# saitejasrivilli/movie-recommender-demo

Measured on AMD Instinct MI355X. Metric: end-to-end recs/sec (1M ads d=256, top-500->10), higher is better.
Workload: dtype f32 (f16x3 emulation: 2 fp16 planes per operand, 3 fp16-MFMA products per MAC, fp32 accumulate)

## Files before the change

### include/amdrec.h

```cpp
#ifndef AMDREC_H
#define AMDREC_H
#include <stddef.h>
#include <stdint.h>

#ifdef __cplusplus
extern "C" {
#endif

#define AMDREC_ABI_VERSION 14
#define AMDREC_MAX_K 2048

int amdrec_abi_version(void);
const char* amdrec_last_error(void);

int amdrec_flat_search_workspace(int64_t nq, int64_t nrows, int k, size_t* bytes );
int amdrec_flat_search(const float* corpus, int64_t nrows, int64_t ld_corpus, int dim,
                       const float* queries, int64_t nq, int64_t ld_queries, int k,
                       int64_t pos_offset, float* out_scores ,
                       int64_t* out_pos , void* workspace, size_t workspace_bytes,
                       int* n_fixup, void* stream);

int amdrec_bf16_rows(const float* x, int64_t rows, int64_t ld, int dim, uint16_t* out ,
                     int64_t ld_out, float* max_norm , void* stream);
int amdrec_flat_search_mixed_workspace(int64_t nq, int64_t nrows, int k, int dim, size_t* bytes );
// ... 201 lines not shown
    const int32_t* table_off;
    const int32_t* cards;
    const float* w_proj;
    const float* b_proj;
    const float* w_proj_user;
    const float* w_proj_ad;
    int32_t ldw_proj_user, ldw_proj_ad;
    amdrec_encoder_layer layers[AMDREC_MAX_LAYERS];
    const float* cross_wt[AMDREC_MAX_LAYERS];
    const float* cross_b[AMDREC_MAX_LAYERS];
    const float* head_w1;
    const float* head_b1;
    const float* head_w2[AMDREC_MAX_TASKS];
    const float* head_b2[AMDREC_MAX_TASKS];
    const float* head_w3[AMDREC_MAX_TASKS];
    const float* head_b3[AMDREC_MAX_TASKS];
    const float* ad_proj_cache;
    int64_t ld_ad_proj_cache;
    const float* ad_hidden_cache;
    int64_t ld_ad_hidden_cache;
    const uint16_t* cross_wt_x6[AMDREC_MAX_LAYERS];
    const uint16_t* head_w1_x6;
    amdrec_x3_weights x3;
} amdrec_ranker_params;

int amdrec_ranker_workspace(const amdrec_ranker_params* p , int64_t rows, size_t* bytes );
int amdrec_ranker_forward(const amdrec_ranker_params* p , const int64_t* user_cat,
                          const float* numerical, int64_t user_rowdiv, const int64_t* ad_cat,
                          const int64_t* ad_rowmap, int64_t rows, float* out_logits, int64_t ld_logits,
                          int* bad_index_flag, int64_t n_user_rows, int64_t n_ad_rows, void* workspace,
                          size_t workspace_bytes, void* stream);

int amdrec_ranker_forward_ctr_first(const amdrec_ranker_params* p , const int64_t* user_cat,
                                    const float* numerical, int64_t user_rowdiv, const int64_t* ad_cat,
                                    const int64_t* ad_rowmap, int64_t rows, float* out_logits ,
                                    int64_t ld_logits, int* bad_index_flag, int64_t n_user_rows, int64_t n_ad_rows,
                                    float* trunk_out , int64_t ld_trunk, void* workspace,
                                    size_t workspace_bytes, void* stream);
int amdrec_ranker_ctr_first_supported(const amdrec_ranker_params* p , int64_t rows);
int amdrec_ranker_winner_heads(const amdrec_ranker_params* p , const float* trunk ,
                               int64_t ld_trunk, int64_t n_trunk_rows, const int32_t* slots ,
                               int64_t n_users, int k_c, int top_k, float* out_scores ,
                               void* workspace, size_t workspace_bytes, void* stream);
int amdrec_ranker_ctr_first_workspace(const amdrec_ranker_params* p , int64_t rows, int64_t n_winner_rows,
                                      size_t* bytes );

// ... 76 lines not shown
```

### movie-recommender-demo_amd/amdrec/ranker.py

```python
from __future__ import annotations

from typing import Dict, List, NamedTuple, Optional, Tuple

import torch
import torch.nn as nn

from . import _lib, weights


class _Attention(nn.Module):
    def __init__(self, d_model, num_heads, dropout):
        super().__init__()
        assert d_model % num_heads == 0
        self.d_model, self.num_heads, self.d_k = d_model, num_heads, d_model // num_heads
        for n in ("W_q", "W_k", "W_v", "W_o"):
            setattr(self, n, nn.Linear(d_model, d_model))
        self.dropout = nn.Dropout(dropout)


class _FFN(nn.Module):
    def __init__(self, d_model, d_ff, dropout):
        super().__init__()
        self.fc1, self.fc2 = nn.Linear(d_model, d_ff), nn.Linear(d_ff, d_model)
        self.dropout = nn.Dropout(dropout)
# ... 49 lines not shown
        super().__init__()
        self.user_embeddings = nn.ModuleDict({n: nn.Embedding(c, embedding_dim) for n, c in user_feature_dims.items()})
        self.ad_embeddings = nn.ModuleDict({n: nn.Embedding(c, embedding_dim) for n, c in ad_feature_dims.items()})
        total = (len(user_feature_dims) + len(ad_feature_dims)) * embedding_dim + numerical_dim
        self.feature_projection = nn.Linear(total, d_model)
        self.positional_encoding = nn.Parameter(torch.randn(1, max_seq_len, d_model))
        self.transformer_layers = nn.ModuleList([_EncoderLayer(d_model, num_heads, d_ff, dropout)
                                                 for _ in range(num_layers)])
        self.feature_interaction = _Cross(d_model, 3, dropout)
        self.prediction_heads = nn.ModuleDict({t: _head(d_model, dropout) for t in ("ctr", "engagement", "revenue")})
        self.d_model = d_model
        self.dropout = nn.Dropout(dropout)
        self._user_names, self._ad_names, self._n_num = list(user_feature_dims), list(ad_feature_dims), numerical_dim
        self._packed = None
        self._ad_cache = None
        self.fuse_attention = True
        self.fold_first_attention = True
        self.cache_first_ffn = True
        self.hidden_cache_max_bytes = 8 << 30
        self.gemm_engine = "f16x3"
        self.x3_min_rows = 1
        self.x3_variant = 16
        self.x3_cs_max_rows = 0

    ENGINES = ("f16x3", "bf16x6", "fp32")
    SMALL_ROWS = 8192

    def x3_fallback_reason(self):
        return weights.x3_ineligible_reason(self.state_dict(), self.fuse_attention)

    def ctr_first_unsupported_reason(self):
        key = (self.gemm_engine, self.fuse_attention, int(self.x3_variant), int(self.x3_min_rows), _lib._REG_EPOCH[0])
        c = self.__dict__.get("_ctr_first_why")
        if c is None or c[0] != key:
            c = self.__dict__["_ctr_first_why"] = (key, self._ctr_first_unsupported_reason())
        return c[1]

    def _ctr_first_unsupported_reason(self):
        if self.gemm_engine != "f16x3":
            return f"gemm_engine {self.gemm_engine!r} (the mode runs on the f16x3 row-owner kernels only)"
        why = self.x3_fallback_reason()
        if why is not None:
            return f"not the row-owner engine's architecture ({why})"
        if int(self.x3_variant) != 16:
            return f"x3_variant {self.x3_variant} (the 32-row kernel has no task window and no gathered input)"
        if int(self.x3_min_rows) != 1:
# ... 99 lines not shown
                out = hid[n_old:]
                _lib.check(lib.amdrec_ranker_project_ads_hidden(
                    _lib.C.byref(params), _lib.ptr(tail), n_new - n_old, _lib.ptr(out), hid.stride(0), _lib.ptr(ws),
                    ws.numel(), _lib.stream_ptr(dev)))
        self._ad_cache = _AdCache(c.key, *_table_key(new_table), proj, hid)

    def _entry_for(self, table) -> Optional[_AdCache]:
        c = getattr(self, "_ad_cache", None)
        if c is None or self._packed is None or c.key != self._packed.key or c[1:4] != _table_key(table):
            return None
        return c

    def _cache_for(self, table):
        return getattr(self._entry_for(table), "proj", None)

    def _hidden_cache_for(self, table):
        return getattr(self._entry_for(table), "hidden", None)

    def _pack(self, device):
        if self.gemm_engine not in self.ENGINES:
            raise ValueError(f"gemm_engine must be one of {self.ENGINES}")
        key = (str(device), self.fuse_attention, bool(self.fold_first_attention), bool(self.cache_first_ffn),
               self.gemm_engine, int(self.x3_min_rows), int(self.x3_variant), int(self.x3_cs_max_rows),
               _lib.tensor_versions(self))
        if self._packed is None or self._packed.key != key:
            sd = self.state_dict()
            why = weights.x3_ineligible_reason(sd, self.fuse_attention) if self.gemm_engine == "f16x3" else None
            x3 = self.gemm_engine == "f16x3" and why is None
            if why is not None:
                import warnings
                warnings.warn(f"amdrec TransformerRanker: gemm_engine 'f16x3' is not available for these weights ({why}); "
                              f"running the generic tile GEMMs (bf16x6 above {self.SMALL_ROWS} rows, fp32 MFMA below)",
                              RuntimeWarning, stacklevel=3)
            self._packed = _Packed(key, *weights.pack_ranker(
                sd, self._user_names, self._ad_names, self._n_num, device, fuse_attention=self.fuse_attention,
                x6=self.gemm_engine == "bf16x6" or (self.gemm_engine == "f16x3" and not x3), x3=x3,
                x3_min_rows=self.x3_min_rows, x3_variant=self.x3_variant, x3_cs_max_rows=self.x3_cs_max_rows,
                fold_first_attention=bool(self.fold_first_attention), cache_first_ffn=bool(self.cache_first_ffn)))
        return self._packed.params, self._packed.tasks

    def load_state_dict(self, state_dict, *a, **k):
        r = super().load_state_dict(state_dict, *a, **k)
        self.invalidate()
        return r

    def autograd_forward(self, user_categorical, ad_categorical, numerical, mask=None):
        import math
        F = torch.nn.functional
        ue = torch.cat([e(user_categorical[:, i].long()) for i, e in enumerate(self.user_embeddings.values())], dim=1)
        ae = torch.cat([e(ad_categorical[:, i].long()) for i, e in enumerate(self.ad_embeddings.values())], dim=1)
        x = self.feature_projection(torch.cat([ue, ae, numerical], dim=1)).unsqueeze(1)
        x = self.dropout(x + self.positional_encoding[:, :1, :])
        for layer in self.transformer_layers:
            at = layer.self_attention
            B = x.size(0)
            q = at.W_q(x).view(B, -1, at.num_heads, at.d_k).transpose(1, 2)
            k = at.W_k(x).view(B, -1, at.num_heads, at.d_k).transpose(1, 2)
            v = at.W_v(x).view(B, -1, at.num_heads, at.d_k).transpose(1, 2)
            scores = torch.matmul(q, k.transpose(-2, -1)) / math.sqrt(at.d_k)
            if mask is not None:
                scores = scores.masked_fill(mask == 0, -1e9)
# ... 150 lines not shown
```

### movie-recommender-demo_amd/amdrec/weights.py

```python
from __future__ import annotations

import ctypes as C
from typing import Dict, List, NamedTuple

import numpy as np
import torch

MAX_LAYERS = 8
MAX_TASKS = 4
_FP = C.c_void_p
TASKS = ("ctr", "engagement", "revenue")


class TowerParams(C.Structure):
    _fields_ = [("n_feat", C.c_int32), ("emb_dim", C.c_int32), ("n_num", C.c_int32), ("n_layers", C.c_int32),
                ("dims", C.c_int32 * (MAX_LAYERS + 1)), ("ldw", C.c_int32 * MAX_LAYERS),
                ("tables", _FP), ("table_off", _FP), ("cards", _FP),
                ("w", _FP * MAX_LAYERS), ("b", _FP * MAX_LAYERS), ("renormalize", C.c_int32)]


class EncoderLayer(C.Structure):
    _fields_ = [(n, _FP) for n in ("w_v", "b_v", "w_o", "b_o", "ln1_g", "ln1_b", "w_1", "b_1", "w_2", "b_2",
                                   "ln2_g", "ln2_b")] + [("ldw_dm", C.c_int32), ("ldw_ff", C.c_int32)] + \
               [(n, _FP) for n in ("w_o_x6", "w_1_x6", "w_2_x6")]
# ... 8 lines not shown
                ("stream_cs", _FP), ("chunks_cs", C.c_int64), ("cs_max_rows", C.c_int64), ("fold_attn1", C.c_int64),
                ("stream_hc", _FP), ("chunks_hc", C.c_int64), ("params_hc", _FP), ("w_user_uq", _FP), ("b_user_uq", _FP),
                ("w_hidden_ad", _FP),
                ("stream_ctr", _FP), ("chunks_ctr", C.c_int64), ("stream_ctr_cs", _FP), ("chunks_ctr_cs", C.c_int64),
                ("stream_ctr_hc", _FP), ("chunks_ctr_hc", C.c_int64), ("stream_win", _FP), ("chunks_win", C.c_int64),
                ("stream_win_cs", _FP), ("chunks_win_cs", C.c_int64)]


class RankerParams(C.Structure):
    _fields_ = [("n_user_feat", C.c_int32), ("n_ad_feat", C.c_int32), ("emb_dim", C.c_int32), ("n_num", C.c_int32),
                ("d_model", C.c_int32), ("d_ff", C.c_int32), ("n_layers", C.c_int32), ("n_cross", C.c_int32),
                ("n_tasks", C.c_int32), ("head_h1", C.c_int32), ("head_h2", C.c_int32), ("ln_eps", C.c_float),
                ("ldw_proj", C.c_int32), ("ldw_cross", C.c_int32), ("ldw_head1", C.c_int32),
                ("ldw_head2", C.c_int32),
                ("tables", _FP), ("table_off", _FP), ("cards", _FP), ("w_proj", _FP), ("b_proj", _FP),
                ("w_proj_user", _FP), ("w_proj_ad", _FP), ("ldw_proj_user", C.c_int32), ("ldw_proj_ad", C.c_int32),
                ("layers", EncoderLayer * MAX_LAYERS),
                ("cross_wt", _FP * MAX_LAYERS), ("cross_b", _FP * MAX_LAYERS),
                ("head_w1", _FP), ("head_b1", _FP),
                ("head_w2", _FP * MAX_TASKS), ("head_b2", _FP * MAX_TASKS),
                ("head_w3", _FP * MAX_TASKS), ("head_b3", _FP * MAX_TASKS),
                ("ad_proj_cache", _FP), ("ld_ad_proj_cache", C.c_int64),
                ("ad_hidden_cache", _FP), ("ld_ad_hidden_cache", C.c_int64),
                ("cross_wt_x6", _FP * MAX_LAYERS), ("head_w1_x6", _FP), ("x3", X3Weights)]


def _np64(t):
    if isinstance(t, torch.Tensor):
        return t.detach().cpu().double().numpy()
    return np.asarray(t, dtype=np.float64)


def split_planes(w32: np.ndarray) -> np.ndarray:
    w = np.ascontiguousarray(w32, dtype=np.float32)
    out_f, ld = w.shape
    assert ld % 32 == 0
    u = w.view(np.uint32)
    h = (u & np.uint32(0xffff0000)).view(np.float32)
    r1 = w - h
    m = (r1.view(np.uint32) & np.uint32(0xffff0000)).view(np.float32)
    r2 = r1 - m
    planes = np.stack([(x.view(np.uint32) >> np.uint32(16)).astype(np.uint16) for x in (h, m, r2)], axis=0)
    assert np.array_equal(h + m + r2, w)
    return np.ascontiguousarray(planes.reshape(3, out_f, ld // 16, 16).transpose(1, 2, 0, 3)).view(np.int16)


X3_TARGET_EXP = 12
# ... 91 lines not shown
    for t in range(T + 1):
        for u in range(8):
            if t < T:
                out += _pair(f1, 2 * t, u)
            if t >= 1:
                out += _pair(f2, 2 * u, t - 1)
    return np.stack(out)


def x3b_stream_ffn_stage2(f2):
    out = []
    for t in range(f2.shape[1]):
        for u in range(8):
            out += _pair(f2, 2 * u, t)
    return np.stack(out)


def _task_window(f2s, tiles_per_task, tasks):
    t0, n = (0, len(f2s)) if tasks is None else tasks
    assert 0 <= t0 and n >= 1 and t0 + n <= len(f2s)
    return f2s[t0:t0 + n], t0 * tiles_per_task


def x3b_stream_heads(f1, f2s, tiles_per_task, tasks=None):
    f2s, base = _task_window(f2s, tiles_per_task, tasks)
    nt = len(f2s) * tiles_per_task
    assert nt % 2 == 0 and (nt * 10) % 4 == 0, "head stream is not a whole number of chunks"
    out = []
    for tt in range(nt + 1):
        prev = tt - 1
        for u in range(8):
            if tt < nt:
                out += _pair(f1, 2 * (base + tt), u)
            if tt >= 1 and u in (3, 7):
                out += _pair(f2s[prev // tiles_per_task], 2 * (u // 4), prev % tiles_per_task)
    return np.stack(out)


def _wave_chunk(groups):
    out = []
    for g in groups:
        out += g if g is not None else [np.zeros((64, 8), np.uint16)] * 4
    assert len(out) == 16
    return out


def x3c_stream_gemm256(fr):
    assert fr.shape[0] == 16
    out = []
    for ks in range(fr.shape[1]):
        for j in range(2):
# ... 83 lines not shown

def x3_hidden_bound(w1: np.ndarray, b1: np.ndarray):
    return float(16.0 * np.linalg.norm(w1, axis=1).max() * (1 + 1e-6)), float(np.abs(b1).max())


def x3_split(mats: Dict, variant: int = 32, fold_first: bool = False):
    mats, lift = x3_rebalance(mats)
    frags = x3_frags if variant == 32 else x3b_frags
    fr, sc = {"tiles": mats["h1"].shape[0] // len(mats["h2"]) // 32}, {}
    for name, dst in (("ov", "sw_ov"), ("w1", "sw_1"), ("w2", "sw_2"), ("cross", "sw_cross")):
        ws = [None if name == "ov" and fold_first and l == 0 else w for l, w in enumerate(mats[name])]
        sc[dst] = [1.0 if w is None else x3_pow2_scale(np.abs(w).max()) for w in ws]
        fr[name] = [None if w is None else frags(w, s) for w, s in zip(ws, sc[dst])]
    sc["sw_h1"] = x3_pow2_scale(np.abs(mats["h1"]).max())
    sc["sw_h2"] = x3_pow2_scale(max(np.abs(w).max() for w in mats["h2"]))
    fr["h1"], fr["h2"] = frags(mats["h1"], sc["sw_h1"]), [frags(w, sc["sw_h2"]) for w in mats["h2"]]
    bounds = [x3_hidden_bound(w, b) for w, b in zip(mats["w1"], mats["b1"])]
    sc["hn"], sc["hb"] = [n for n, _ in bounds], [b for _, b in bounds]
    sc["hn_head"], sc["hb_head"] = x3_hidden_bound(mats["h1"], mats["hb1"])
    sc["lift"] = lift
    return fr, sc


def x3_order(fr: Dict, kind, cache_first_ffn: bool = False, tasks=None, trunk: bool = True) -> np.ndarray:
    s_gemm, s_cross, s_ffn, s_heads = _X3_ORDER[kind]
    assert trunk or not cache_first_ffn
    assert tasks is None or kind in (16, "16cs"), "task windows exist for the 16-row kernels only"
    parts = []
    for l, (ov, f1, f2) in enumerate(zip(fr["ov"], fr["w1"], fr["w2"]) if trunk else ()):
        parts += [] if ov is None else [s_gemm(ov)]
        parts.append(x3b_stream_ffn_stage2(f2) if cache_first_ffn and l == 0 else s_ffn(f1, f2))
    parts += [s_cross(f) for f in fr["cross"]] if trunk else []
    parts.append(s_heads(fr["h1"], fr["h2"], fr["tiles"], *(() if tasks is None else (tasks,))))
    stream = np.concatenate(parts)
    assert stream.shape[0] % 16 == 0 and (kind != "16cs" or all(len(q) % 64 == 0 for q in parts))
    return stream


def x3_ctr_first_orders(n_tasks: int, column_split: bool, cache_first_ffn: bool) -> Dict:
    win = (1, n_tasks - 1)
    orders = {"ctr": dict(kind=16, tasks=(0, 1)), "win": dict(kind=16, tasks=win, trunk=False)}
    if column_split:
        orders["ctr_cs"] = dict(kind="16cs", tasks=(0, 1))
        orders["win_cs"] = dict(kind="16cs", tasks=win, trunk=False)
    if cache_first_ffn:
        orders["ctr_hc"] = dict(kind=16, tasks=(0, 1), cache_first_ffn=True)
    return orders


def pack_x3_stream(mats: Dict, variant: int = 32, fold_first: bool = False, cache_first_ffn: bool = False) -> Dict:
    assert variant in (16, 32, "16cs")
    assert not cache_first_ffn or (variant == 16 and fold_first)
    fr, sc = x3_split(mats, variant, fold_first)
    stream = x3_order(fr, variant, cache_first_ffn)
    return {"stream": stream, "chunks": stream.shape[0] // 16, **sc}

# ... 184 lines not shown
        L.w_o, L.ldw_dm, L.w_o_x6 = pk.mat(c["wov"], x6)
    else:
        L.b_v = pk.vec(c["bv"])
        L.w_v, L.ldw_dm, _ = pk.mat(c["wv"])
        L.w_o, L.ldw_dm, L.w_o_x6 = pk.mat(c["wo"], x6)
    L.w_1, L.ldw_dm, L.w_1_x6 = pk.mat(c["w1"], x6)
    L.b_o = pk.vec(c["b_ov"] if fuse_attention else c["bo"])
    L.w_2, L.ldw_ff, L.w_2_x6 = pk.mat(c["w2"], x6)
    for dst, src in (("b_1", "b1"), ("b_2", "b2"), ("ln1_g", "g1"), ("ln1_b", "be1"), ("ln2_g", "g2"), ("ln2_b", "be2")):
        setattr(L, dst, pk.vec(c[src]))


def _pack_x3(p: RankerParams, pk: Packed, ch: RankerChain, wproj, bproj, nu: int, na: int, cache_first_ffn: bool):
    f32 = lambda a: a.astype(np.float32).astype(np.float64)
    fold = bool(p.x3.fold_attn1)
    mats = {"ov": [f32(L["wov"]) for L in ch.layers], "w1": [f32(L["w1"]) for L in ch.layers],
            "b1": [f32(L["b1"]) for L in ch.layers], "w2": [f32(L["w2"]) for L in ch.layers],
            "cross": [f32(w) for w in ch.cross_wt], "h1": f32(ch.head_w1), "hb1": f32(ch.head_b1),
            "h2": [f32(h["w2"]) for h in ch.heads]}
    fr, sc = x3_split(mats, p.x3.variant, fold)
    pk.x3_fragments = fr

    def stream(kind, **kw):
        s = x3_order(fr, kind, **kw)
        return pk.ptr(s.view(np.int16)), s.shape[0] // 16
    lift = sc["lift"]
    layers = [dict(L, b1=_scaled(L["b1"], f)) for L, f in zip(ch.layers, lift["w1"])]
    heads = [dict(h, b2=_scaled(h["b2"], f), w3=_scaled(h["w3"], 1.0 / f)) for h, f in zip(ch.heads, lift["h2"])]
    blob = pack_x3_params(layers, ch.cross_b, _scaled(ch.head_b1, lift["h1"]), heads, fold_first=fold)
    assert len(blob) <= X3_PARAM_FLOATS
    p.x3.params, p.x3.n_params = pk.ptr(blob), len(blob)
    p.x3.stream, p.x3.chunks = stream(p.x3.variant)
    if p.x3.cs_max_rows >= 0 and x3c_available(p):
        p.x3.stream_cs, p.x3.chunks_cs = stream("16cs")
    if cache_first_ffn and x3_hidden_cache(p):
        hc = first_ffn_cache(ch, nu, na, folded=(wproj, bproj), lift=lift["w1"][0])
        p.x3.stream_hc, p.x3.chunks_hc = stream(16, cache_first_ffn=True)
        blob_hc = blob.copy()
        blob_hc[512:512 + len(hc["c"])] = hc["c"].astype(np.float32)
        p.x3.params_hc = pk.ptr(blob_hc)
        p.x3.w_user_uq, ldu, _ = pk.mat(np.concatenate([_user_ad_columns(wproj, nu, na)[0], hc["w_user"]]))
        p.x3.b_user_uq = pk.vec(np.concatenate([bproj, hc["b"]]))
        p.x3.w_hidden_ad, lda, _ = pk.mat(hc["w_ad"])
        assert ldu == p.ldw_proj_user and lda == p.ldw_proj_ad
    for dst in ("sw_ov", "sw_1", "sw_2", "hn", "hb", "sw_cross"):
        for i, v in enumerate(sc[dst]):
            getattr(p.x3, dst)[i] = v
    p.x3.sw_h1, p.x3.sw_h2, p.x3.hn_head, p.x3.hb_head = sc["sw_h1"], sc["sw_h2"], sc["hn_head"], sc["hb_head"]


def ctr_first_packable(p: RankerParams) -> bool:
    return bool(p.x3.stream) and p.x3.variant == 16 and p.n_tasks >= 2


def pack_ctr_first(p: RankerParams, pk: Packed) -> bool:
    if p.x3.stream_ctr:
        return True
    fr = getattr(pk, "x3_fragments", None)
    if fr is None or not ctr_first_packable(p):
        return False
    for stem, kw in x3_ctr_first_orders(p.n_tasks, bool(p.x3.stream_cs), bool(p.x3.stream_hc)).items():
        s = x3_order(fr, **kw)
        setattr(p.x3, "stream_" + stem, pk.ptr(s.view(np.int16)))
        setattr(p.x3, "chunks_" + stem, s.shape[0] // 16)
    return True


def pack_ranker(sd: Dict, user_names: List[str], ad_names: List[str], n_num: int, device, ln_eps=1e-5,
                fuse_attention: bool = True, x6: bool = True, x3: bool = False, x3_min_rows: int = 0,
                x3_variant: int = 32, x3_cs_max_rows: int = 0, fold_first_attention: bool = False,
                cache_first_ffn: bool = False):
    pk = Packed(device)
    tables = [sd[f"user_embeddings.{n}.weight"] for n in user_names] + \
             [sd[f"ad_embeddings.{n}.weight"] for n in ad_names]
    p = RankerParams()
    p.tables, p.table_off, p.cards, emb_dim = pack_tables(pk, tables)
    ch = ranker_chain(sd)
    if len(ch.layers) > MAX_LAYERS:
        raise ValueError(f"at most {MAX_LAYERS} encoder layers are supported (num_layers > {MAX_LAYERS})")
    x3 = bool(x3) and x3_eligible(sd, fuse_attention)
    fold = bool(fold_first_attention and x3 and int(x3_min_rows) == 1 and ch.layers)
    wproj, bproj = folded_projection(ch) if fold else (ch.w_proj, ch.b_proj)
    assert wproj.shape[1] == len(tables) * emb_dim + n_num
    p.n_user_feat, p.n_ad_feat, p.emb_dim, p.n_num = len(user_names), len(ad_names), emb_dim, n_num
    p.d_model, p.ln_eps = wproj.shape[0], ln_eps
    p.w_proj, p.ldw_proj, _ = pk.mat(wproj)
    nu, na = len(user_names) * emb_dim, len(ad_names) * emb_dim
    if nu + n_num > 0 and na > 0:
        w_user, w_ad = _user_ad_columns(wproj, nu, na)
        p.w_proj_user, p.ldw_proj_user, _ = pk.mat(w_user)
        p.w_proj_ad, p.ldw_proj_ad, _ = pk.mat(w_ad)
    p.b_proj = pk.vec(bproj)
    for l, c in enumerate(ch.layers):
        _pack_encoder_layer(p.layers[l], pk, c, fuse_attention, x6)
    p.n_layers, p.n_cross, p.n_tasks = len(ch.layers), len(ch.cross_wt), len(ch.tasks)
    p.d_ff = ch.layers[-1]["w1"].shape[0] if ch.layers else 4
    for c, (w, b) in enumerate(zip(ch.cross_wt, ch.cross_b)):
        p.cross_wt[c], p.ldw_cross, p.cross_wt_x6[c] = pk.mat(w, x6)
        p.cross_b[c] = pk.vec(b)
    p.head_h1, p.head_h2 = ch.head_w1.shape[0] // len(ch.tasks), ch.heads[0]["w2"].shape[0]
    p.head_w1, p.ldw_head1, p.head_w1_x6 = pk.mat(ch.head_w1, x6)
    p.head_b1 = pk.vec(ch.head_b1)
    for i, h in enumerate(ch.heads):
        p.head_w2[i], p.ldw_head2, _ = pk.mat(h["w2"])
        p.head_b2[i], p.head_w3[i], p.head_b3[i] = pk.vec(h["b2"]), pk.vec(h["w3"]), pk.vec(h["b3"])
    if x3:
        p.x3.variant, p.x3.fold_attn1 = x3_variant, int(fold)
        p.x3.min_rows, p.x3.cs_max_rows = int(x3_min_rows), int(x3_cs_max_rows)
        _pack_x3(p, pk, ch, wproj, bproj, nu, na, cache_first_ffn)
    return p, pk, ch.tasks
```

### movie-recommender-demo_amd/csrc/ranker_x3.hip

```cpp
#include "rowowner.hpp"
#include "rowowner16.hpp"
#include "rowowner16c.hpp"
#include "../../include/amdrec.h"

using namespace amdrec;

static bool x3_folded(const amdrec_ranker_params* p) { return p->x3.fold_attn1 != 0; }
static long long x3_param_floats(const amdrec_ranker_params* p) {
    const long long n = (long long)p->n_layers * (6 * 256 + p->d_ff) + 256ll * p->n_cross + (long long)p->n_tasks * (p->head_h1 + 132) -
                        (x3_folded(p) ? 256 : 0);
    return (n + 1023) / 1024 * 1024;
}

static bool x3_eligible(const amdrec_ranker_params* p) {
    if (p->x3.stream == nullptr || p->x3.chunks <= 0 || p->x3.params == nullptr) return false;
    if (p->x3.variant != 16 && p->x3.variant != 32) return false;
    if (x3_param_floats(p) > x3::PARAM_FLOATS) return false;
    if (p->d_model != 256 || (p->n_layers > 0 && p->d_ff % 32 != 0) || p->head_h1 % 32 != 0 || p->head_h2 != 64) return false;
    if (2 * p->n_layers + p->n_cross + 1 > x3::MAX_PHASES || p->n_tasks > 4) return false;
    for (int l = 0; l < p->n_layers; ++l)
        if (p->layers[l].w_v != nullptr) return false;
    if (x3_folded(p) && (p->n_layers < 1 || p->x3.min_rows != 1)) return false;
    return true;
}

static bool x3c_available(const amdrec_ranker_params* p) {
    return p->x3.variant == 16 && p->x3.stream_cs != nullptr && p->x3.chunks_cs > 0 &&
           (p->n_layers == 0 || p->d_ff % 128 == 0) && p->head_h1 % 128 == 0;
}

constexpr long long X3B4_MAX_ROWS = 256ll * 64;

enum class X3Shape { Rows32x128, Rows16x128, Rows16x64, ColSplit };
static X3Shape x3_shape(const amdrec_ranker_params* p, long long rows) {
    const long long cs_rows = p->x3.cs_max_rows > 0 ? p->x3.cs_max_rows : (p->x3.cs_max_rows < 0 ? 0 : x3c::MAX_ROWS);
    if (x3c_available(p) && rows <= cs_rows) return X3Shape::ColSplit;
    if (p->x3.variant != 16) return X3Shape::Rows32x128;
    return rows <= X3B4_MAX_ROWS ? X3Shape::Rows16x64 : X3Shape::Rows16x128;
}

static bool x3_hidden_cache(const amdrec_ranker_params* p, X3Shape shape) {
    return x3_folded(p) && shape == X3Shape::Rows16x128 && p->x3.stream_hc != nullptr && p->x3.chunks_hc > 0 &&
// ... 30 lines not shown
        if (l == 0 && fold) {
            A.type = x3::PH_LN; A.gamma = o; A.beta = o + 256; A.sw1 = 1.f; A.sw2 = 1.f; A.ln_eps = p->ln_eps;
            o += 512;
        } else {
            A.type = x3::PH_ATTN_LN; A.b1 = o; A.gamma = o + 256; A.beta = o + 512; A.sw1 = p->x3.sw_ov[l];
            A.sw2 = 1.f; A.ln_eps = p->ln_eps;
            o += 768;
        }
        x3::Phase& F = G.ph[n++];
        F.type = hc && l == 0 ? x3::PH_FFN_LN_CACHED : x3::PH_FFN_LN; F.n_steps = p->d_ff / 32; F.b1 = o; F.b2 = o + p->d_ff; F.gamma = o + p->d_ff + 256;
        F.beta = o + p->d_ff + 512;
        F.sw1 = p->x3.sw_1[l]; F.sw2 = p->x3.sw_2[l]; F.hn = p->x3.hn[l]; F.hb = p->x3.hb[l]; F.ln_eps = p->ln_eps;
        o += p->d_ff + 768;
    }
    for (int c = 0; c < p->n_cross; ++c) {
        if (win.heads_only) { o += 256; continue; }
        x3::Phase& C = G.ph[n++];
        C.type = x3::PH_CROSS; C.b1 = o; C.sw1 = p->x3.sw_cross[c]; C.sw2 = 1.f;
        o += 256;
    }
    x3::Phase& H = G.ph[n++];
    H.type = x3::PH_HEADS; H.n_steps = p->head_h1 / 32; H.n_tasks = win.n_tasks; H.b1 = o + win.first_task * p->head_h1;
    H.sw1 = p->x3.sw_h1; H.sw2 = p->x3.sw_h2; H.hn = p->x3.hn_head; H.hb = p->x3.hb_head;
    o += p->n_tasks * p->head_h1;
    for (int t = 0; t < p->n_tasks; ++t) {
        const int i = t - win.first_task;
        if (i >= 0 && i < win.n_tasks) { G.hb2[i] = o; G.hw3[i] = o + 64; G.hb3[i] = o + 128; }
        o += 132;
    }
    REQUIRE(p->x3.n_params == x3_param_floats(p), "x3: parameter blob has %lld floats, the architecture needs %lld",
            (long long)p->x3.n_params, x3_param_floats(p));
    G.params = hc ? p->x3.params_hc : p->x3.params;
    G.n_params = (int)p->x3.n_params;
    const long long per_layer = 16 + 4ll * (p->d_ff / 32);
    const long long hidden_tiles = (long long)win.n_tasks * (p->head_h1 / 32);
    const long long heads = cs ? hidden_tiles * 3 : hidden_tiles * 40 / 16;
    REQUIRE(cs || hidden_tiles * 40 % 16 == 0, "x3: head stream is not a whole number of chunks");
    REQUIRE(!cs || hidden_tiles % 4 == 0, "x3: column-split head stream is not a whole number of super-steps");
    const long long trunk = p->n_layers * per_layer - (fold ? 16 : 0) - (hc ? 2ll * (p->d_ff / 32) : 0) + 16ll * p->n_cross;
    const long long total = (win.heads_only ? 0 : trunk) + heads;
    const amdrec_x3_weights& w = p->x3;
    const void* stream = all_tasks ? (cs ? w.stream_cs : (hc ? w.stream_hc : w.stream))
                         : ctr_first ? (cs ? w.stream_ctr_cs : (hc ? w.stream_ctr_hc : w.stream_ctr))
                                     : (cs ? w.stream_win_cs : w.stream_win);
    const long long have = all_tasks ? (cs ? w.chunks_cs : (hc ? w.chunks_hc : w.chunks))
                           : ctr_first ? (cs ? w.chunks_ctr_cs : (hc ? w.chunks_ctr_hc : w.chunks_ctr))
                                       : (cs ? w.chunks_win_cs : w.chunks_win);
    REQUIRE(stream != nullptr, "x3: the stream of this program is not packed");
    REQUIRE(total == have, "x3: stream length %lld chunks does not match the architecture (%lld)", have, total);
    G.n_phases = n_phases < 0 || n_phases > n ? n : n_phases;
    G.total_chunks = (int)total;
    G.stream = reinterpret_cast<const unsigned char*>(stream);
    return AMDREC_OK;
}

static double x3_weight_elements(const x3::Program& G) {
    double w = 0;
    for (int i = 0; i < G.n_phases; ++i) {
        const x3::Phase& P = G.ph[i];
        if (P.type == x3::PH_ATTN_LN || P.type == x3::PH_CROSS) w += 256.0 * 256.0;
// ... 206 lines not shown
```

### movie-recommender-demo_amd/csrc/rowowner16_impl.hpp

```cpp

#pragma clang diagnostic push
#pragma clang diagnostic ignored "-Wuninitialized-const-reference"
namespace amdrec {
namespace AMDREC_X3B_NAMESPACE {

using x3::CHUNK_BYTES, x3::CHUNK_FRAGS, x3::DBG, x3::f16x8, x3::FRAG_BYTES, x3::Input, x3::lds_byte, x3::lds_cfloat, x3::Phase,
    x3::Program, x3::RING_BYTES;
using x16::add_rows, x16::group6, x16::hidden_planes, x16::init_pair, x16::layer_norm, x16::layer_norm_scaled, x16::load_rows,
    x16::param4, x16::prepare, x16::reduce_sum4, x16::row_scale, x16::split8, x16::store_rows;

#if !defined(AMDREC_X3B_WAVES) || !defined(AMDREC_X3B_NAMESPACE)
#error "include rowowner16.hpp, not this file"
#endif
constexpr int WAVES = AMDREC_X3B_WAVES, ROWS_PER_WAVE = 16, ROWS_PER_WG = WAVES * ROWS_PER_WAVE;
constexpr int DMA_PER_WAVE = CHUNK_FRAGS / WAVES;
constexpr bool PAIRED = WAVES == 8 && !(DBG & (256 | 512));
constexpr int NBUF = PAIRED ? x3::NBUF - 1 : x3::NBUF, DEPTH = NBUF - 3;
constexpr int PAIR_BYTES = CHUNK_BYTES / 4;
constexpr int DMA_GROUP = 1;

struct Ring {
    lds_byte* lds_dma;
    lds_byte* lds_rd;
    int issued, total;
// ... 488 lines not shown

template <bool S1, bool S2, int P0, int GI>
__device__ __forceinline__ void heads_groups(Ring& ring, f16x8 (&cur)[4], const f16x8 (&xh)[8], const f16x8 (&xl)[8],
                                             f32x4& a10, f32x4& a11, f32x4 (&acc2)[4], const f16x8& hh, const f16x8& hl) {
    constexpr int NG = (S1 ? 8 : 0) + (S2 ? 2 : 0);
    constexpr bool is2 = S2 && (!S1 || GI == 4 || GI == 9);
    constexpr int u = !S1 ? 0 : (S2 ? (GI < 4 ? GI : GI - 1) : GI);
    constexpr int pr = !S1 ? GI : (GI == 9 ? 1 : 0);
    f16x8 nxt[4];
    if constexpr (GI < NG - 1) ring.read4<(P0 + GI + 1) & 3>(nxt);
    ring.timed_landed(cur);
    if constexpr (is2) group6(cur, hh, hl, acc2[2 * pr], acc2[2 * pr + 1]);
    else group6(cur, xh[u], xl[u], a10, a11);
    if constexpr (GI < NG - 1) heads_groups<S1, S2, P0, GI + 1>(ring, nxt, xh, xl, a10, a11, acc2, hh, hl);
}
template <bool S1, bool S2, int P0>
__device__ __forceinline__ void heads_step(Ring& ring, const f16x8 (&xh)[8], const f16x8 (&xl)[8], f32x4& a10, f32x4& a11,
                                           f32x4 (&acc2)[4], const f16x8& hh, const f16x8& hl) {
    f16x8 cur[4];
    ring.read4<P0>(cur);
    heads_groups<S1, S2, P0, 0>(ring, cur, xh, xl, a10, a11, acc2, hh, hl);
}

__device__ __forceinline__ void phase_heads(Ring& ring, const Program& G, const Phase& P, const f32x4 (&x)[16], float* out,
                                            long long ld_out, long long row, bool row_ok, int g, lds_cfloat* pb) {
    float s, inv;
    row_scale(x, s, inv);
    f16x8 xh[8], xl[8];
#pragma unroll
    for (int ks = 0; ks < 8; ++ks) split8(x[2 * ks], x[2 * ks + 1], s, xh[ks], xl[ks]);
    const float sh = x3::hidden_scale(fmaf(P.hn * 8192.0f, inv, P.hb));
    const float b1s = s * P.sw1, c1 = sh * inv / P.sw1, un2 = 1.0f / (P.sw2 * sh), lim1 = 60000.f / c1;
    const int T = P.n_steps, NT = P.n_tasks * T;
    f32x4 acc2[4], a10, a11;
    f16x8 hh, hl;
    init_pair(acc2[0], acc2[1], pb, G.hb2[0], 0, P.sw2 * sh);
    init_pair(acc2[2], acc2[3], pb, G.hb2[0], 2, P.sw2 * sh);
    init_pair(a10, a11, pb, P.b1, 0, b1s);
    heads_step<true, false, 0>(ring, xh, xl, a10, a11, acc2, hh, hl);
    const float probe = a10[0];
    int task = 0, t_in = 0;
    for (int tt = 1; tt <= NT; ++tt) {
        hidden_planes(a10, a11, c1, lim1, hh, hl);
        if (tt < NT) {
            init_pair(a10, a11, pb, P.b1, 2 * tt, b1s);
            if (tt & 1) heads_step<true, true, 0>(ring, xh, xl, a10, a11, acc2, hh, hl);
            else heads_step<true, true, 2>(ring, xh, xl, a10, a11, acc2, hh, hl);
        } else {
            heads_step<false, true, 2>(ring, xh, xl, a10, a11, acc2, hh, hl);
        }
        if (++t_in == T) {
            float dot = 0.f;
#pragma unroll
            for (int t = 0; t < 4; ++t) {
                const f32x4 w = param4(pb, G.hw3[task], t);
#pragma unroll
                for (int r = 0; r < 4; ++r) dot += fmaxf(acc2[t][r] * un2, 0.f) * w[r];
            }
            dot = reduce_sum4(dot);
            if (g == 0 && row_ok) out[(long long)task * ld_out + row] = x3::keep_nan(dot + pb[G.hb3[task]], probe);
            t_in = 0;
            if (++task < P.n_tasks) {
                init_pair(acc2[0], acc2[1], pb, G.hb2[task], 0, P.sw2 * sh);
                init_pair(acc2[2], acc2[3], pb, G.hb2[task], 2, P.sw2 * sh);
            }
        }
    }
}

__device__ __forceinline__ void run_chain(const Program& G, const Input& in, long long rows, float* scratch, float* x_out,
                                          long long ld_xout, float* logits, long long ld_logits, unsigned char* smem, int wave,
                                          int lane, lds_cfloat* pb) {
    const int g = lane >> 4, q = lane & 15;
    const long long row = (long long)blockIdx.x * ROWS_PER_WG + wave * ROWS_PER_WAVE + q;
    const bool row_ok = row < rows;
    const long long rowc = row_ok ? row : rows - 1;
    Ring ring;
    const unsigned long long t_begin = (DBG & 16) ? __builtin_amdgcn_s_memtime() : 0ull;
    ring.start(G.stream, G.total_chunks, (lds_byte*)smem, wave, lane);

    f32x4 x[16];
    if (in.X != nullptr) {
        load_rows(x, in.X + x3::dense_row(in, rowc) * in.ldx, g);
    } else {
        const long long gr = in.row_base + rowc;
        long long a = in.rowmap ? in.rowmap[gr] : gr;
        a = a < 0 ? 0 : (a >= in.n_cache ? in.n_cache - 1 : a);
        load_rows(x, in.cache + a * in.ldc, g);
        add_rows(x, in.U + (gr / in.rowdiv) * in.ldu, g);
    }
// ... 10 lines not shown
                else phase_ffn_ln_role_b(ring, P, x, pb, box);
            } else {
                phase_ffn_ln(ring, P, x, pb);
            }
        }
        else if (type == x3::PH_LN) rstd = layer_norm(x, pb, P.gamma, P.beta, P.ln_eps);
        else if (WAVES == 8 && type == x3::PH_FFN_LN_CACHED) {
            if constexpr (WAVES == 8) {
                const long long gr = in.row_base + rowc;
                long long a = in.rowmap ? in.rowmap[gr] : gr;
                a = a < 0 ? 0 : (a >= in.n_cache ? in.n_cache - 1 : a);
                phase_ffn_ln_cached(ring, P, x, rstd, in.hcache + a * in.ldh + 4 * g, in.Q + (gr / in.rowdiv) * in.ldu + 4 * g,
                                    pb);
            }
        } else break;
    }
    if (p < G.n_phases && __builtin_amdgcn_readfirstlane(G.ph[p].type) == x3::PH_CROSS) {
        f32x4 x0[16];
#pragma unroll
        for (int t = 0; t < 16; ++t) x0[t] = x[t];
        for (; p < G.n_phases && __builtin_amdgcn_readfirstlane(G.ph[p].type) == x3::PH_CROSS; ++p)
            phase_cross(ring, G.ph[p], x, x0, pb);
    }
    if (p < G.n_phases) phase_heads(ring, G, G.ph[p], x, logits, ld_logits, row, row_ok, g, pb);
    if (x_out != nullptr && row_ok) store_rows(x, x_out + row * ld_xout, g);
    ring.drain();
    if ((DBG & 16) && lane == 0) {
        float* dbg = logits + 3 * ld_logits + ((long long)blockIdx.x * WAVES + wave) * 4;
        dbg[0] = (float)(__builtin_amdgcn_s_memtime() - t_begin);
        dbg[1] = (DBG & 32) ? (float)ring.t_lds : (float)ring.t_wait;
        dbg[2] = (DBG & 32) ? (float)ring.t_cal : (float)ring.t_bar;
        dbg[3] = (float)ring.t_dma;
    }
}

__global__ __launch_bounds__(64 * WAVES, 2) void ranker_x3b_kernel(Program G, Input in, long long rows, float* scratch,
                                                            float* x_out, long long ld_xout, float* logits,
                                                            long long ld_logits) {
    extern __shared__ __attribute__((aligned(16))) unsigned char smem[];
    const int tid = threadIdx.x, lane = tid & 63;
    const int wave = __builtin_amdgcn_readfirstlane(tid >> 6);
    const int g = lane >> 4;

    lds_byte* pbase = (lds_byte*)smem + RING_BYTES;
    for (int o = 0; o + wave * 1024 < G.n_params * 4; o += WAVES * 1024)
        __builtin_amdgcn_global_load_lds((const __attribute__((address_space(1))) void*)(
                                             reinterpret_cast<const unsigned char*>(G.params) + o + tid * 16),
                                         (__attribute__((address_space(3))) void*)(pbase + o + wave * 1024), 16, 0, 0);
// ... 9 lines not shown
```

### movie-recommender-demo_amd/csrc/x3_common.hpp

```cpp
#pragma once
#include "common.hpp"

namespace amdrec {
namespace x3 {

typedef _Float16 f16x8 __attribute__((ext_vector_type(8)));
typedef float f32x8 __attribute__((ext_vector_type(8)));
typedef __attribute__((address_space(3))) const float lds_cfloat;
typedef __attribute__((address_space(3))) unsigned char lds_byte;

constexpr int FRAG_BYTES = 1024;
constexpr int CHUNK_FRAGS = 16;
constexpr int CHUNK_BYTES = CHUNK_FRAGS * FRAG_BYTES;
#ifndef AMDREC_X3_NBUF
#define AMDREC_X3_NBUF 7
#endif
constexpr int NBUF = AMDREC_X3_NBUF;
constexpr int PARAM_FLOATS = 11264;
constexpr int RING_BYTES = NBUF * CHUNK_BYTES;
constexpr int DEPTH = NBUF - 3;
constexpr int TARGET_EXP = 12;

enum PhaseType { PH_ATTN_LN = 0, PH_FFN_LN = 1, PH_CROSS = 2, PH_HEADS = 3, PH_LN = 4, PH_FFN_LN_CACHED = 5 };

struct Phase {
    int type;
    int n_steps;
    int n_tasks;
    int pad_;
    int b1;
    int b2;
    int gamma;
    int beta;
    float sw1, sw2;
    float hn, hb;
    float ln_eps;
    float pad2_;
};
constexpr int MAX_PHASES = 20;
struct Program {
    int n_phases;
    int total_chunks;
    const unsigned char* stream;
    const float* params;
    int n_params;
    int hb2[4];
    int hw3[4];
    int hb3[4];
    Phase ph[MAX_PHASES];
};

struct Input {
// ... 43 lines not shown
```

Measured before the change: 184,400.

## Reorder head weight stream task-major with fully unrolled per-task head pipeline

```diff
diff --git a/include/amdrec.h b/include/amdrec.h
--- a/include/amdrec.h
+++ b/include/amdrec.h
@@ -247,6 +247,7 @@
     const uint16_t* cross_wt_x6[AMDREC_MAX_LAYERS];
     const uint16_t* head_w1_x6;
     amdrec_x3_weights x3;
+    int64_t x3_heads_task_major;
 } amdrec_ranker_params;
 
 int amdrec_ranker_workspace(const amdrec_ranker_params* p , int64_t rows, size_t* bytes );
diff --git a/movie-recommender-demo_amd/amdrec/ranker.py b/movie-recommender-demo_amd/amdrec/ranker.py
--- a/movie-recommender-demo_amd/amdrec/ranker.py
+++ b/movie-recommender-demo_amd/amdrec/ranker.py
@@ -95,6 +95,7 @@
         self.x3_min_rows = 1
         self.x3_variant = 16
         self.x3_cs_max_rows = 0
+        self.heads_task_major = True
 
     ENGINES = ("f16x3", "bf16x6", "fp32")
     SMALL_ROWS = 8192
@@ -240,7 +241,7 @@
             raise ValueError(f"gemm_engine must be one of {self.ENGINES}")
         key = (str(device), self.fuse_attention, bool(self.fold_first_attention), bool(self.cache_first_ffn),
                self.gemm_engine, int(self.x3_min_rows), int(self.x3_variant), int(self.x3_cs_max_rows),
-               _lib.tensor_versions(self))
+               bool(self.heads_task_major), _lib.tensor_versions(self))
         if self._packed is None or self._packed.key != key:
             sd = self.state_dict()
             why = weights.x3_ineligible_reason(sd, self.fuse_attention) if self.gemm_engine == "f16x3" else None
@@ -254,7 +255,8 @@
                 sd, self._user_names, self._ad_names, self._n_num, device, fuse_attention=self.fuse_attention,
                 x6=self.gemm_engine == "bf16x6" or (self.gemm_engine == "f16x3" and not x3), x3=x3,
                 x3_min_rows=self.x3_min_rows, x3_variant=self.x3_variant, x3_cs_max_rows=self.x3_cs_max_rows,
-                fold_first_attention=bool(self.fold_first_attention), cache_first_ffn=bool(self.cache_first_ffn)))
+                fold_first_attention=bool(self.fold_first_attention), cache_first_ffn=bool(self.cache_first_ffn),
+                heads_task_major=bool(self.heads_task_major)))
         return self._packed.params, self._packed.tasks
 
     def load_state_dict(self, state_dict, *a, **k):
diff --git a/movie-recommender-demo_amd/amdrec/weights.py b/movie-recommender-demo_amd/amdrec/weights.py
--- a/movie-recommender-demo_amd/amdrec/weights.py
+++ b/movie-recommender-demo_amd/amdrec/weights.py
@@ -54,7 +54,7 @@
                 ("head_w3", _FP * MAX_TASKS), ("head_b3", _FP * MAX_TASKS),
                 ("ad_proj_cache", _FP), ("ld_ad_proj_cache", C.c_int64),
                 ("ad_hidden_cache", _FP), ("ld_ad_hidden_cache", C.c_int64),
-                ("cross_wt_x6", _FP * MAX_LAYERS), ("head_w1_x6", _FP), ("x3", X3Weights)]
+                ("cross_wt_x6", _FP * MAX_LAYERS), ("head_w1_x6", _FP), ("x3", X3Weights), ("x3_heads_task_major", C.c_int64)]
 
 
 def _np64(t):
@@ -192,11 +192,29 @@
     return f2s[t0:t0 + n], t0 * tiles_per_task
 
 
-def x3b_stream_heads(f1, f2s, tiles_per_task, tasks=None):
+X3B_HEADS_MAX_TILES = 8
+
+
+def x3_heads_task_major(tiles_per_task: int) -> bool:
+    return tiles_per_task % 2 == 0 and tiles_per_task <= X3B_HEADS_MAX_TILES
+
+
+def x3b_stream_heads(f1, f2s, tiles_per_task, tasks=None, task_major=False):
     f2s, base = _task_window(f2s, tiles_per_task, tasks)
+    out = []
+    if task_major and x3_heads_task_major(tiles_per_task):
+        for task, f2 in enumerate(f2s):
+            first = base + task * tiles_per_task
+            for t in range(tiles_per_task):
+                for u in range(8):
+                    out += _pair(f1, 2 * (first + t), u)
+            for t in range(tiles_per_task):
+                for pr in range(2):
+                    out += _pair(f2, 2 * pr, t)
+        assert len(out) % (16 * len(f2s)) == 0, "a task of the head stream is not a whole number of chunks"
+        return np.stack(out)
     nt = len(f2s) * tiles_per_task
     assert nt % 2 == 0 and (nt * 10) % 4 == 0, "head stream is not a whole number of chunks"
-    out = []
     for tt in range(nt + 1):
         prev = tt - 1
         for u in range(8):
@@ -326,7 +344,8 @@
     return fr, sc
 
 
-def x3_order(fr: Dict, kind, cache_first_ffn: bool = False, tasks=None, trunk: bool = True) -> np.ndarray:
+def x3_order(fr: Dict, kind, cache_first_ffn: bool = False, tasks=None, trunk: bool = True,
+             heads_task_major: bool = False) -> np.ndarray:
     s_gemm, s_cross, s_ffn, s_heads = _X3_ORDER[kind]
     assert trunk or not cache_first_ffn
     assert tasks is None or kind in (16, "16cs"), "task windows exist for the 16-row kernels only"
@@ -335,7 +354,8 @@
         parts += [] if ov is None else [s_gemm(ov)]
         parts.append(x3b_stream_ffn_stage2(f2) if cache_first_ffn and l == 0 else s_ffn(f1, f2))
     parts += [s_cross(f) for f in fr["cross"]] if trunk else []
-    parts.append(s_heads(fr["h1"], fr["h2"], fr["tiles"], *(() if tasks is None else (tasks,))))
+    parts.append(s_heads(fr["h1"], fr["h2"], fr["tiles"], *(() if tasks is None else (tasks,)),
+                         **({"task_major": True} if heads_task_major and kind == 16 else {})))
     stream = np.concatenate(parts)
     assert stream.shape[0] % 16 == 0 and (kind != "16cs" or all(len(q) % 64 == 0 for q in parts))
     return stream
@@ -566,7 +586,7 @@
     pk.x3_fragments = fr
 
     def stream(kind, **kw):
-        s = x3_order(fr, kind, **kw)
+        s = x3_order(fr, kind, heads_task_major=bool(p.x3_heads_task_major), **kw)
         return pk.ptr(s.view(np.int16)), s.shape[0] // 16
     lift = sc["lift"]
     layers = [dict(L, b1=_scaled(L["b1"], f)) for L, f in zip(ch.layers, lift["w1"])]
@@ -604,7 +624,7 @@
     if fr is None or not ctr_first_packable(p):
         return False
     for stem, kw in x3_ctr_first_orders(p.n_tasks, bool(p.x3.stream_cs), bool(p.x3.stream_hc)).items():
-        s = x3_order(fr, **kw)
+        s = x3_order(fr, heads_task_major=bool(p.x3_heads_task_major), **kw)
         setattr(p.x3, "stream_" + stem, pk.ptr(s.view(np.int16)))
         setattr(p.x3, "chunks_" + stem, s.shape[0] // 16)
     return True
@@ -613,7 +633,7 @@
 def pack_ranker(sd: Dict, user_names: List[str], ad_names: List[str], n_num: int, device, ln_eps=1e-5,
                 fuse_attention: bool = True, x6: bool = True, x3: bool = False, x3_min_rows: int = 0,
                 x3_variant: int = 32, x3_cs_max_rows: int = 0, fold_first_attention: bool = False,
-                cache_first_ffn: bool = False):
+                cache_first_ffn: bool = False, heads_task_major: bool = False):
     pk = Packed(device)
     tables = [sd[f"user_embeddings.{n}.weight"] for n in user_names] + \
              [sd[f"ad_embeddings.{n}.weight"] for n in ad_names]
@@ -651,5 +671,6 @@
     if x3:
         p.x3.variant, p.x3.fold_attn1 = x3_variant, int(fold)
         p.x3.min_rows, p.x3.cs_max_rows = int(x3_min_rows), int(x3_cs_max_rows)
+        p.x3_heads_task_major = int(bool(heads_task_major) and x3_variant == 16 and x3_heads_task_major(p.head_h1 // 32))
         _pack_x3(p, pk, ch, wproj, bproj, nu, na, cache_first_ffn)
     return p, pk, ch.tasks
diff --git a/movie-recommender-demo_amd/csrc/ranker_x3.hip b/movie-recommender-demo_amd/csrc/ranker_x3.hip
--- a/movie-recommender-demo_amd/csrc/ranker_x3.hip
+++ b/movie-recommender-demo_amd/csrc/ranker_x3.hip
@@ -11,6 +11,13 @@
                         (x3_folded(p) ? 256 : 0);
     return (n + 1023) / 1024 * 1024;
 }
+
+static bool x3_heads_task_major_fits(const amdrec_ranker_params* p) {
+    const int tiles = p->head_h1 / 32;
+    static_assert(x3b::HEADS_MAX_TILES == x3b4::HEADS_MAX_TILES, "one rule for both workgroup shapes");
+    return p->x3.variant == 16 && tiles % 2 == 0 && tiles <= x3b::HEADS_MAX_TILES;
+}
+static bool x3_heads_task_major(const amdrec_ranker_params* p) { return p->x3_heads_task_major != 0; }
 
 static bool x3_eligible(const amdrec_ranker_params* p) {
     if (p->x3.stream == nullptr || p->x3.chunks <= 0 || p->x3.params == nullptr) return false;
@@ -18,6 +25,7 @@
     if (x3_param_floats(p) > x3::PARAM_FLOATS) return false;
     if (p->d_model != 256 || (p->n_layers > 0 && p->d_ff % 32 != 0) || p->head_h1 % 32 != 0 || p->head_h2 != 64) return false;
     if (2 * p->n_layers + p->n_cross + 1 > x3::MAX_PHASES || p->n_tasks > 4) return false;
+    if (x3_heads_task_major(p) && !x3_heads_task_major_fits(p)) return false;
     for (int l = 0; l < p->n_layers; ++l)
         if (p->layers[l].w_v != nullptr) return false;
     if (x3_folded(p) && (p->n_layers < 1 || p->x3.min_rows != 1)) return false;
@@ -94,6 +102,7 @@
     x3::Phase& H = G.ph[n++];
     H.type = x3::PH_HEADS; H.n_steps = p->head_h1 / 32; H.n_tasks = win.n_tasks; H.b1 = o + win.first_task * p->head_h1;
     H.sw1 = p->x3.sw_h1; H.sw2 = p->x3.sw_h2; H.hn = p->x3.hn_head; H.hb = p->x3.hb_head;
+    H.task_major = !cs && x3_heads_task_major(p);
     o += p->n_tasks * p->head_h1;
     for (int t = 0; t < p->n_tasks; ++t) {
         const int i = t - win.first_task;
@@ -107,7 +116,8 @@
     const long long per_layer = 16 + 4ll * (p->d_ff / 32);
     const long long hidden_tiles = (long long)win.n_tasks * (p->head_h1 / 32);
     const long long heads = cs ? hidden_tiles * 3 : hidden_tiles * 40 / 16;
-    REQUIRE(cs || hidden_tiles * 40 % 16 == 0, "x3: head stream is not a whole number of chunks");
+    REQUIRE(cs || H.task_major || hidden_tiles * 40 % 16 == 0, "x3: head stream is not a whole number of chunks");
+    REQUIRE(!H.task_major || (p->head_h1 / 32) * 40 % 32 == 0, "x3: a task of the head stream is not a whole number of chunks");
     REQUIRE(!cs || hidden_tiles % 4 == 0, "x3: column-split head stream is not a whole number of super-steps");
     const long long trunk = p->n_layers * per_layer - (fold ? 16 : 0) - (hc ? 2ll * (p->d_ff / 32) : 0) + 16ll * p->n_cross;
     const long long total = (win.heads_only ? 0 : trunk) + heads;
diff --git a/movie-recommender-demo_amd/csrc/rowowner16_impl.hpp b/movie-recommender-demo_amd/csrc/rowowner16_impl.hpp
--- a/movie-recommender-demo_amd/csrc/rowowner16_impl.hpp
+++ b/movie-recommender-demo_amd/csrc/rowowner16_impl.hpp
@@ -534,8 +534,93 @@
     heads_groups<S1, S2, P0, 0>(ring, cur, xh, xl, a10, a11, acc2, hh, hl);
 }
 
-__device__ __forceinline__ void phase_heads(Ring& ring, const Program& G, const Phase& P, const f32x4 (&x)[16], float* out,
+template <int J>
+__device__ __forceinline__ void hidden_planes2(const f32x4& a0, const f32x4& a1, float c, float lim, f16x8& hh, f16x8& hl) {
+    static_assert(J >= 0 && J < 8 && J % 2 == 0, "a pair of elements");
+    if (DBG & 8) {
+        if (J == 0) asm volatile("" : "+v"(hh), "+v"(hl) : "v"(a0), "v"(a1));
+        return;
+    }
+#pragma unroll
+    for (int j = J; j < J + 2; ++j) {
+        const float v = __builtin_amdgcn_fmed3f(j < 4 ? a0[j & 3] : a1[j & 3], 0.f, lim) * c;
+        const _Float16 h = (_Float16)v;
+        hh[j] = h;
+        hl[j] = (_Float16)(v - (float)h);
+    }
+}
+__device__ __forceinline__ void heads_logit(const Program& G, int task, const f32x4 (&acc2)[4], float un2, float probe, float* out,
                                             long long ld_out, long long row, bool row_ok, int g, lds_cfloat* pb) {
+    float dot = 0.f;
+#pragma unroll
+    for (int t = 0; t < 4; ++t) {
+        const f32x4 w = param4(pb, G.hw3[task], t);
+#pragma unroll
+        for (int r = 0; r < 4; ++r) dot += fmaxf(acc2[t][r] * un2, 0.f) * w[r];
+    }
+    dot = reduce_sum4(dot);
+    if (g == 0 && row_ok) out[(long long)task * ld_out + row] = x3::keep_nan(dot + pb[G.hb3[task]], probe);
+}
+
+constexpr int HEADS_MAX_TILES = 8;
+template <int NTL, int J>
+__device__ __forceinline__ void heads_last_ahead(const f32x4 (&a)[2][2], float c1, float lim1, f16x8& hh, f16x8& hl) {
+    if constexpr (NTL >= 4) {
+        if constexpr (J < 4) hidden_planes2<2 * J>(a[1][0], a[1][1], c1, lim1, hh, hl);
+    } else if constexpr (J < 2) {
+        hidden_planes2<4 * J>(a[1][0], a[1][1], c1, lim1, hh, hl);
+        hidden_planes2<4 * J + 2>(a[1][0], a[1][1], c1, lim1, hh, hl);
+    }
+}
+template <int NTL, int J>
+__device__ __forceinline__ void heads2_groups(Ring& ring, f16x8 (&cur)[4], const f32x4 (&a)[2][2], float c1, float lim1,
+                                              f16x8 (&hh)[HEADS_MAX_TILES], f16x8 (&hl)[HEADS_MAX_TILES], f32x4 (&acc2)[4]) {
+    f16x8 nxt[4];
+    if constexpr (J < 2 * NTL - 1) ring.read4<(J + 1) & 3>(nxt);
+    ring.timed_landed(cur);
+    group6(cur, hh[J >> 1], hl[J >> 1], acc2[2 * (J & 1)], acc2[2 * (J & 1) + 1]);
+    heads_last_ahead<NTL, J>(a, c1, lim1, hh[NTL - 1], hl[NTL - 1]);
+    if constexpr (J < 2 * NTL - 1) heads2_groups<NTL, J + 1>(ring, nxt, a, c1, lim1, hh, hl, acc2);
+}
+template <int I, int GI>
+__device__ __forceinline__ void heads1_groups(Ring& ring, f16x8 (&cur)[4], const f16x8 (&xh)[8], const f16x8 (&xl)[8],
+                                              f32x4 (&a)[2][2], float c1, float lim1, f16x8 (&hh)[HEADS_MAX_TILES],
+                                              f16x8 (&hl)[HEADS_MAX_TILES], lds_cfloat* pb, int b1, int tile0, float b1s) {
+    f16x8 nxt[4];
+    if constexpr (GI < 7) ring.read4<(GI + 1) & 3>(nxt);
+    ring.timed_landed(cur);
+    group6(cur, xh[GI], xl[GI], a[I & 1][0], a[I & 1][1]);
+    if constexpr (I >= 1 && GI >= 1 && GI <= 4)
+        hidden_planes2<2 * (GI - 1)>(a[(I - 1) & 1][0], a[(I - 1) & 1][1], c1, lim1, hh[I - 1], hl[I - 1]);
+    if constexpr (GI == 5 && I + 1 < HEADS_MAX_TILES)
+        init_pair(a[(I + 1) & 1][0], a[(I + 1) & 1][1], pb, b1, 2 * (tile0 + I + 1), b1s);
+    if constexpr (GI < 7) heads1_groups<I, GI + 1>(ring, nxt, xh, xl, a, c1, lim1, hh, hl, pb, b1, tile0, b1s);
+}
+template <int I>
+__device__ __forceinline__ void heads_task(Ring& ring, const f16x8 (&xh)[8], const f16x8 (&xl)[8], f32x4 (&a)[2][2], float c1,
+                                           float lim1, f16x8 (&hh)[HEADS_MAX_TILES], f16x8 (&hl)[HEADS_MAX_TILES],
+                                           f32x4 (&acc2)[4], lds_cfloat* pb, int b1, int tile0, float b1s, int T,
+                                           float& probe) {
+    f16x8 cur[4];
+    ring.read4<0>(cur);
+    heads1_groups<I, 0>(ring, cur, xh, xl, a, c1, lim1, hh, hl, pb, b1, tile0, b1s);
+    if constexpr (I == 0) probe = tile0 == 0 ? a[0][0][0] : probe;
+    if constexpr ((I & 1) == 0) {
+        heads_task<I + 1>(ring, xh, xl, a, c1, lim1, hh, hl, acc2, pb, b1, tile0, b1s, T, probe);
+    } else {
+        if (I + 1 < HEADS_MAX_TILES && I + 1 < T) {
+            if constexpr (I + 1 < HEADS_MAX_TILES)
+                heads_task<I + 1>(ring, xh, xl, a, c1, lim1, hh, hl, acc2, pb, b1, tile0, b1s, T, probe);
+        } else {
+            ring.read4<0>(cur);
+            heads2_groups<I + 1, 0>(ring, cur, a, c1, lim1, hh, hl, acc2);
+        }
+    }
+}
+
+__device__ __forceinline__ bool phase_heads(Ring& ring, const Program& G, const Phase& P, const f32x4 (&x)[16], float* x_out,
+                                            long long ld_xout, float* out, long long ld_out, long long row, bool row_ok, int g,
+                                            lds_cfloat* pb) {
     float s, inv;
     row_scale(x, s, inv);
     f16x8 xh[8], xl[8];
@@ -544,7 +629,22 @@
     const float sh = x3::hidden_scale(fmaf(P.hn * 8192.0f, inv, P.hb));
     const float b1s = s * P.sw1, c1 = sh * inv / P.sw1, un2 = 1.0f / (P.sw2 * sh), lim1 = 60000.f / c1;
     const int T = P.n_steps, NT = P.n_tasks * T;
-    f32x4 acc2[4], a10, a11;
+    f32x4 acc2[4];
+    if (P.task_major) {
+        if (x_out != nullptr && row_ok) store_rows(x, x_out + row * ld_xout, g);
+        f32x4 a[2][2];
+        f16x8 hh[HEADS_MAX_TILES], hl[HEADS_MAX_TILES];
+        float probe = 0.f;
+        for (int task = 0; task < P.n_tasks; ++task) {
+            init_pair(acc2[0], acc2[1], pb, G.hb2[task], 0, P.sw2 * sh);
+            init_pair(acc2[2], acc2[3], pb, G.hb2[task], 2, P.sw2 * sh);
+            init_pair(a[0][0], a[0][1], pb, P.b1, 2 * task * T, b1s);
+            heads_task<0>(ring, xh, xl, a, c1, lim1, hh, hl, acc2, pb, P.b1, task * T, b1s, T, probe);
+            heads_logit(G, task, acc2, un2, probe, out, ld_out, row, row_ok, g, pb);
+        }
+        return true;
+    }
+    f32x4 a10, a11;
     f16x8 hh, hl;
     init_pair(acc2[0], acc2[1], pb, G.hb2[0], 0, P.sw2 * sh);
     init_pair(acc2[2], acc2[3], pb, G.hb2[0], 2, P.sw2 * sh);
@@ -562,15 +662,7 @@
             heads_step<false, true, 2>(ring, xh, xl, a10, a11, acc2, hh, hl);
         }
         if (++t_in == T) {
-            float dot = 0.f;
-#pragma unroll
-            for (int t = 0; t < 4; ++t) {
-                const f32x4 w = param4(pb, G.hw3[task], t);
-#pragma unroll
-                for (int r = 0; r < 4; ++r) dot += fmaxf(acc2[t][r] * un2, 0.f) * w[r];
-            }
-            dot = reduce_sum4(dot);
-            if (g == 0 && row_ok) out[(long long)task * ld_out + row] = x3::keep_nan(dot + pb[G.hb3[task]], probe);
+            heads_logit(G, task, acc2, un2, probe, out, ld_out, row, row_ok, g, pb);
             t_in = 0;
             if (++task < P.n_tasks) {
                 init_pair(acc2[0], acc2[1], pb, G.hb2[task], 0, P.sw2 * sh);
@@ -578,6 +670,7 @@
             }
         }
     }
+    return false;
 }
 
 __device__ __forceinline__ void run_chain(const Program& G, const Input& in, long long rows, float* scratch, float* x_out,
@@ -634,8 +727,9 @@
         for (; p < G.n_phases && __builtin_amdgcn_readfirstlane(G.ph[p].type) == x3::PH_CROSS; ++p)
             phase_cross(ring, G.ph[p], x, x0, pb);
     }
-    if (p < G.n_phases) phase_heads(ring, G, G.ph[p], x, logits, ld_logits, row, row_ok, g, pb);
-    if (x_out != nullptr && row_ok) store_rows(x, x_out + row * ld_xout, g);
+    bool stored = false;
+    if (p < G.n_phases) stored = phase_heads(ring, G, G.ph[p], x, x_out, ld_xout, logits, ld_logits, row, row_ok, g, pb);
+    if (!stored && x_out != nullptr && row_ok) store_rows(x, x_out + row * ld_xout, g);
     ring.drain();
     if ((DBG & 16) && lane == 0) {
         float* dbg = logits + 3 * ld_logits + ((long long)blockIdx.x * WAVES + wave) * 4;
diff --git a/movie-recommender-demo_amd/csrc/x3_common.hpp b/movie-recommender-demo_amd/csrc/x3_common.hpp
--- a/movie-recommender-demo_amd/csrc/x3_common.hpp
+++ b/movie-recommender-demo_amd/csrc/x3_common.hpp
@@ -27,7 +27,7 @@
     int type;
     int n_steps;
     int n_tasks;
-    int pad_;
+    int task_major;
     int b1;
     int b2;
     int gamma;
```

New measurement: 184,800 (median of 4 runs). About the same (+0.2%).
